# ViliamVadocz/takzero

Hardware: AMD Instinct MI355X
Metric: mcts_simulations_per_s (higher is better)
Workload: dtype f16

## Files before the change

### takzero_amd/csrc/tz_nn.hip

```cpp
#include "tz_nn.h"
#include "tz_fp8.h"
#include "tz_fp6.h"
#include <type_traits>
#include "tz_ot.h"

#include <algorithm>
#include <cmath>
#include <cstdio>
#include <cstdlib>
#include <cstring>
#include <atomic>
#include <map>
#include <memory>
#include <mutex>
#include <thread>

int tz_nn_launch_split(int sp, int n, const void* net_args, int max_positions, hipStream_t st);
int tz_nn_launch_c6(int n, const void* net_args, int max_positions, hipStream_t st);
size_t tz_nn_c6_seed_bytes(int n, int max_positions);

namespace {

typedef float f32x4 __attribute__((ext_vector_type(4)));
typedef unsigned int u32x4 __attribute__((ext_vector_type(4)));
// ... 2623 lines not shown
                                const float wv = W(co, ci, t);
                                const _Float16 hi = (_Float16)wv;
                                const size_t at = (((((size_t)t * m_total + mh) * ct_total + ct) * 2) * 64 + lane) * 32 + i;
                                p8[at] = tz_f32_to_e4m3((wv - (float)hi) * 2048.0f * sw);
                                p8[at + 64 * 32] = tz_f32_to_e4m3((float)hi * sw);
                            }
                        }
            if ((rc = upload(p8, &L->w8))) return rc;
        }
        if (with_c6) {
            if (L->cin_pad % 128) return tz_fail(TZ_EINVAL, "weights: TZ_PREC_F16C6 needs input channels in multiples of 128");
            const int g_total = L->cin_pad / 128;
            constexpr size_t REC = 3328;
            std::vector<unsigned char> p6((size_t)taps * g_total * ct_total * REC, 0);
            for (int t = 0; t < taps; t++)
                for (int g = 0; g < g_total; g++)
                    for (int ct = 0; ct < ct_total; ct++) {
                        unsigned char* rec = p6.data() + (((size_t)t * g_total + g) * ct_total + ct) * REC;
                        for (int lane = 0; lane < 64; lane++) {
                            const int co = ct * 16 + (lane & 15), q = lane >> 4;
                            float lo[32], hi[32], amax_l = 0.0f, amax_h = 0.0f;
                            for (int i = 0; i < 32; i++) {
                                const int ci = 128 * g + 32 * (i >> 3) + 8 * q + (i & 7);
                                const float wv = (co < cout && ci < cin) ? W(co, ci, t) : 0.0f;
                                const _Float16 h = (_Float16)wv;
                                hi[i] = (float)h;
                                lo[i] = wv - (float)h;
                                amax_h = std::max(amax_h, fabsf(hi[i]));
                                amax_l = std::max(amax_l, fabsf(lo[i]));
                            }
                            const uint32_t bl = tz_e2m3_block_scale_byte(amax_l), bh = tz_e2m3_block_scale_byte(amax_h);
                            uint8_t cl[32], ch[32];
                            for (int i = 0; i < 32; i++) {
                                cl[i] = tz_f32_to_e2m3(ldexpf(lo[i], 127 - (int)bl));
                                ch[i] = tz_f32_to_e2m3(ldexpf(hi[i], 127 - (int)bh));
                            }
                            uint32_t sl[6], sh[6];
                            tz_pack_fp6x32(cl, sl);
                            tz_pack_fp6x32(ch, sh);
                            memcpy(rec + 0 * 1536 + lane * 16, sl, 16);
                            memcpy(rec + 0 * 1536 + 1024 + lane * 8, sl + 4, 8);
                            memcpy(rec + 1 * 1536 + lane * 16, sh, 16);
                            memcpy(rec + 1 * 1536 + 1024 + lane * 8, sh + 4, 8);
                            const uint32_t sw = bl | (bh << 8);
                            memcpy(rec + 3072 + lane * 4, &sw, 4);
                        }
                    }
            if ((rc = upload(p6, &L->w8))) return rc;
        }
        return upload(p, &L->w_mfma);
    }
    std::vector<float> f((size_t)taps * cin * cout);
    for (int t = 0; t < taps; t++)
        for (int ci = 0; ci < cin; ci++)
            for (int co = 0; co < cout; co++) f[((size_t)t * cin + ci) * cout + co] = W(co, ci, t);
    return upload(f, &L->w_f32);
}

void free_layer(ConvW* L) {
    if (L->w_mfma) (void)hipFree(L->w_mfma);
    if (L->w_lo) (void)hipFree(L->w_lo);
    if (L->w8) (void)hipFree(L->w8);
    if (L->w_f32) (void)hipFree(L->w_f32);
    if (L->bias) (void)hipFree(L->bias);
    *L = ConvW();
}

int bn_fold(const TensorMap& m, const std::string& p, int c, std::vector<float>& scale, std::vector<float>& bias) {
    std::vector<float> g, b, mean, var;
    int rc;
    if ((rc = get_tensor(m, p + ".weight", c, g))) return rc;
    if ((rc = get_tensor(m, p + ".bias", c, b))) return rc;
    if ((rc = get_tensor(m, p + ".running_mean", c, mean))) return rc;
    if ((rc = get_tensor(m, p + ".running_var", c, var))) return rc;
    scale.resize(c);
    bias.resize(c);
    for (int i = 0; i < c; i++) {
        const float s = g[i] / sqrtf(var[i] + 1e-5f);
        scale[i] = s;
        bias[i] = b[i] - mean[i] * s;
    }
    return TZ_OK;
}

struct NetWeights {
    ConvW conv_in, policy;
    std::vector<ConvW> res;
    uint16_t* tower_w = nullptr;
    uint16_t* tower_w_lo = nullptr;
    unsigned char* tower_w8 = nullptr;
    float* c8_scales = nullptr;
    float* tower_bias = nullptr;
    float* heads = nullptr;
    ConvW rnd[2][3];
    uint16_t* rndw[3] = {nullptr, nullptr, nullptr};
    float* rndb[3] = {nullptr, nullptr, nullptr};
    float rnd_min = 0.f, rnd_max = 1.f;
    float* simhash = nullptr;
};

void free_weights(NetWeights& w) {
    free_layer(&w.conv_in);
    free_layer(&w.policy);
    for (auto& l : w.res) free_layer(&l);
    w.res.clear();
    if (w.tower_w) (void)hipFree(w.tower_w);
    if (w.tower_w_lo) (void)hipFree(w.tower_w_lo);
    if (w.tower_w8) (void)hipFree(w.tower_w8);
    if (w.c8_scales) (void)hipFree(w.c8_scales);
    if (w.tower_bias) (void)hipFree(w.tower_bias);
    w.tower_w = nullptr;
    w.tower_w_lo = nullptr;
    w.tower_w8 = nullptr;
    w.c8_scales = nullptr;
    w.tower_bias = nullptr;
    if (w.heads) (void)hipFree(w.heads);
    w.heads = nullptr;
    for (int a = 0; a < 2; a++)
        for (int b = 0; b < 3; b++) free_layer(&w.rnd[a][b]);
    for (int l = 0; l < 3; l++) {
        if (w.rndw[l]) (void)hipFree(w.rndw[l]);
        if (w.rndb[l]) (void)hipFree(w.rndb[l]);
        w.rndw[l] = nullptr;
        w.rndb[l] = nullptr;
    }
    if (w.simhash) (void)hipFree(w.simhash);
    w.simhash = nullptr;
}

int build_weights(tz_net* net, const TensorMap& m, NetWeights& W) {
    const int nn = net->nn, cin = net->cin, prec = net->precision;
    std::vector<float> w, scale, bias;
    int rc;
    if ((rc = get_tensor(m, "core.input_conv2d.weight", (size_t)FILTERS * cin * 9, w))) return rc;
    if ((rc = bn_fold(m, "core.batch_norm", FILTERS, scale, bias))) return rc;
    const bool split = prec == TZ_PREC_F16X2, c8 = prec == TZ_PREC_F16C8, c6 = prec == TZ_PREC_F16C6;
    std::vector<int> c6_perm(FILTERS);
    for (int pos = 0; pos < FILTERS; pos++) c6_perm[pos] = c6_channel_at(pos);
    const std::vector<int>* tower_perm = c6 ? &c6_perm : nullptr;
    if ((rc = build_layer(prec, 9, cin, FILTERS, 256, w, scale, bias, nullptr, &W.conv_in, split || c8 || c6))) return rc;
    W.res.resize(2 * net->blocks);
    {
        const int nl = 2 * net->blocks;
        const int workers = std::max(1, std::min(nl, std::min(16, (int)std::thread::hardware_concurrency())));
        std::atomic<int> next{0}, failed{TZ_OK};
        std::string first_error;
        std::mutex mu;
        const bool background = g_upload_stream != nullptr;
        auto work = [&]() {
            if (hipSetDevice(net->device) != hipSuccess) {
                failed = TZ_EDEVICE;
                return;
            }
            std::unique_ptr<UploadStream> upload_stream(background ? new UploadStream() : nullptr);
            if (upload_stream && !upload_stream->mine) {
                std::lock_guard<std::mutex> lk(mu);
                if (failed == TZ_OK) {
                    failed = TZ_EDEVICE;
                    first_error = "weights: cannot create an upload stream for a build thread";
                }
                return;
            }
            std::vector<float> lw, lscale, lbias;
            for (int l = next++; l < nl && failed == TZ_OK; l = next++) {
                const std::string p = "core.res_block_" + std::to_string(l / 2) + ((l & 1) ? ".b" : ".a");
                int r = get_tensor(m, p + ".conv2d.weight", (size_t)FILTERS * FILTERS * 9, lw);
                if (!r) r = bn_fold(m, p + ".batch_norm", FILTERS, lscale, lbias);
                if (!r) r = build_layer(prec, 9, FILTERS, FILTERS, 256, lw, lscale, lbias, tower_perm, &W.res[l], split, c8, c6);
                if (r) {
                    std::lock_guard<std::mutex> lk(mu);
                    if (failed == TZ_OK) {
                        failed = r;
                        first_error = tz_last_error();
                    }
                }
            }
        };
        std::vector<std::thread> pool;
        for (int t = 1; t < workers; t++) pool.emplace_back(work);
        work();
        for (auto& t : pool) t.join();
        if (failed != TZ_OK) return tz_fail(failed, first_error.empty() ? "weights: a tower layer could not be built" : first_error);
    }
    if (prec != TZ_PREC_F32 && net->blocks > 0) {
        const size_t layer_elems = (size_t)9 * 8 * 16 * 64 * 8, nl = W.res.size();
        TZ_HIP(hipMalloc(&W.tower_w, nl * layer_elems * 2));
        if (split) TZ_HIP(hipMalloc(&W.tower_w_lo, nl * layer_elems * 2));
        const size_t layer_bytes8 = c6 ? (size_t)9 * 2 * 16 * 3328 : (size_t)9 * 2 * 16 * 2 * 64 * 32;
        if (c8 || c6) TZ_HIP(hipMalloc(&W.tower_w8, nl * layer_bytes8));
        TZ_HIP(hipMalloc(&W.tower_bias, nl * FILTERS * sizeof(float)));
        for (size_t l = 0; l < nl; l++) {
            if ((rc = copy_sync(W.tower_w + l * layer_elems, W.res[l].w_mfma, layer_elems * 2, hipMemcpyDeviceToDevice))) return rc;
            if (split && (rc = copy_sync(W.tower_w_lo + l * layer_elems, W.res[l].w_lo, layer_elems * 2, hipMemcpyDeviceToDevice))) return rc;
            if ((c8 || c6) && (rc = copy_sync(W.tower_w8 + l * layer_bytes8, W.res[l].w8, layer_bytes8, hipMemcpyDeviceToDevice))) return rc;
            if ((rc = copy_sync(W.tower_bias + l * FILTERS, W.res[l].bias, FILTERS * sizeof(float), hipMemcpyDeviceToDevice))) return rc;
        }
    }
    if ((rc = get_tensor(m, "policy.conv2d.weight", (size_t)net->pol_ch * FILTERS * 9, w))) return rc;
    if ((rc = get_tensor(m, "policy.conv2d.bias", net->pol_ch, bias))) return rc;
    if ((rc = build_layer(prec, 9, FILTERS, net->pol_ch, net->pol_stride, w, {}, bias, tower_perm, &W.policy, split, c8, c6))) return rc;
    if (c8) {
        std::vector<float> cs;
        for (auto& l : W.res) cs.push_back(l.c8_scale);
        cs.push_back(W.policy.c8_scale);
        if ((rc = upload(cs, &W.c8_scales))) return rc;
    }
    std::vector<float> hv, hu, lv, lu, t1;
    if ((rc = get_tensor(m, "value.conv2d.weight", FILTERS, hv))) return rc;
    if ((rc = get_tensor(m, "ube.conv2d.weight", FILTERS, hu))) return rc;
    if ((rc = get_tensor(m, "value.linear.weight", nn, lv))) return rc;
    if ((rc = get_tensor(m, "ube.linear.weight", nn, lu))) return rc;
    std::vector<float> hw;
    hw.insert(hw.end(), hv.begin(), hv.end());
    hw.insert(hw.end(), hu.begin(), hu.end());
    hw.insert(hw.end(), lv.begin(), lv.end());
    hw.insert(hw.end(), lu.begin(), lu.end());
    for (const char* nm : {"value.conv2d.bias", "ube.conv2d.bias", "value.linear.bias", "ube.linear.bias"}) {
        if ((rc = get_tensor(m, nm, 1, t1))) return rc;
        hw.push_back(t1[0]);
    }
    if ((rc = upload(hw, &W.heads))) return rc;
    if (net->has_rnd) {
        const int in_size = cin * nn;
        std::vector<int> perm(in_size);
        for (int px = 0; px < nn; px++)
            for (int c = 0; c < cin; c++) perm[px * cin + c] = c * nn + px;
        const char* nets[2] = {"rnd_learning", "rnd_target"};
        const char* layers[3] = {"input_linear", "hidden_linear", "final_linear"};
        const int dims[4] = {in_size, 1024, 1024, 512};
        for (int a = 0; a < 2; a++)
            for (int l = 0; l < 3; l++) {
                const std::string p = std::string(nets[a]) + "." + layers[l];
                if ((rc = get_tensor(m, p + ".weight", (size_t)dims[l + 1] * dims[l], w))) return rc;
                if ((rc = get_tensor(m, p + ".bias", dims[l + 1], bias))) return rc;
                if ((rc = build_layer(prec, 1, dims[l], dims[l + 1], 256, w, {}, bias, l == 0 ? &perm : nullptr, &W.rnd[a][l])))
                    return rc;
            }
        if (prec != TZ_PREC_F32) {
            std::vector<float> wa, wb, ba, bb;
            if ((rc = get_tensor(m, "rnd_learning.input_linear.weight", (size_t)1024 * in_size, wa))) return rc;
            if ((rc = get_tensor(m, "rnd_target.input_linear.weight", (size_t)1024 * in_size, wb))) return rc;
            if ((rc = get_tensor(m, "rnd_learning.input_linear.bias", 1024, ba))) return rc;
            if ((rc = get_tensor(m, "rnd_target.input_linear.bias", 1024, bb))) return rc;
            wa.insert(wa.end(), wb.begin(), wb.end());
            ba.insert(ba.end(), bb.begin(), bb.end());
            ConvW cat;
            if ((rc = build_layer(prec, 1, in_size, 2048, 256, wa, {}, ba, &perm, &cat))) return rc;
            W.rndw[0] = cat.w_mfma;
            W.rndb[0] = cat.bias;
            for (int l = 1; l < 3; l++) {
                const size_t welems = (size_t)(W.rnd[0][l].cin_pad / 32) * (W.rnd[0][l].cout_pad / 16) * 512;
                const size_t belems = W.rnd[0][l].cout_pad;
                TZ_HIP(hipMalloc(&W.rndw[l], 2 * welems * 2));
                TZ_HIP(hipMalloc(&W.rndb[l], 2 * belems * sizeof(float)));
                for (int a = 0; a < 2; a++) {
                    if ((rc = copy_sync(W.rndw[l] + a * welems, W.rnd[a][l].w_mfma, welems * 2, hipMemcpyDeviceToDevice))) return rc;
                    if ((rc = copy_sync(W.rndb[l] + a * belems, W.rnd[a][l].bias, belems * sizeof(float), hipMemcpyDeviceToDevice))) return rc;
                }
            }
        }
        if ((rc = get_tensor(m, "min", 1, t1))) return rc;
        W.rnd_min = t1[0];
        if ((rc = get_tensor(m, "max", 1, t1))) return rc;
        W.rnd_max = t1[0];
    }
    if (net->has_hash) {
        if ((rc = get_tensor(m, "simhash_matrix", (size_t)cin * nn * 32, w))) return rc;
        if ((rc = upload(w, &W.simhash))) return rc;
    }
    return TZ_OK;
}

__host__ __device__ constexpr int ppt_small(int nb) { return nb == 1 ? 64 : nb == 3 ? 7 : nb == 4 ? 6 : nb == 5 ? 4 : 3; }

int conv_cfg() {
    static int cfg = -1;
    if (cfg < 0) {
        const char* e = getenv("TZ_CONV_CFG");
        cfg = e ? atoi(e) : 0;
    }
    return cfg;
}

template <int NB, int P, int NW, int RN, int TAPS, bool FROM_STATE, bool SINGLE, int ABL = 0, int LAYOUT = 1, typename ET = __bf16, int OCC = 2>
int launch_conv(const ConvArgs& a, int max_positions, int n_blocks_y, hipStream_t st) {
    constexpr int NN = NB * NB, RT = (P * NN + 15) / 16, LROWS = RT * 16 + 8;
    const size_t smem = LdsImg<LAYOUT>::bytes(LROWS);
    auto kern = conv_mfma_kernel<NB, P, RN, TAPS, FROM_STATE, ABL, SINGLE, NW, LAYOUT, ET, OCC>;
    static bool attr_done[64] = {};
    int attr_dev = 0;
    TZ_HIP(hipGetDevice(&attr_dev));
    bool& attr_set = attr_done[attr_dev & 63];
    if (!attr_set) {
        TZ_HIP(hipFuncSetAttribute(reinterpret_cast<const void*>(kern), hipFuncAttributeMaxDynamicSharedMemorySize, (int)smem));
        attr_set = true;
    }
    dim3 grid((max_positions + P - 1) / P, n_blocks_y, a.groups > 1 ? a.groups : 1);
    hipLaunchKernelGGL(kern, grid, dim3(NW * 64), smem, st, a);
    hipError_t e = hipGetLastError();
    if (e != hipSuccess) return tz_fail(TZ_EDEVICE, std::string("conv launch: ") + hipGetErrorString(e));
    return TZ_OK;
}

int linear_grouped_bf16(int precision, const uint16_t* w, const float* bias, int groups, int cin_pad, int cout_pad, const void* in,
                        int in_stride, int in_z, void* out, int out_stride, int out_z, bool relu, bool out_f32,
                        const int32_t* count_dev, int count_host, int max_positions, hipStream_t st) {
    ConvArgs a;
    memset(&a, 0, sizeof a);
    a.in = in;
    a.count_dev = count_dev;
    a.count_host = count_host;
    a.w = w;
    a.bias = bias;
    a.out = out;
    a.cin_pad = cin_pad;
    a.kc_total = cin_pad / 32;
    a.ct_total = cout_pad / 16;
    a.out_stride = out_stride;
    a.cin_real = cin_pad;
    a.relu = relu;
    a.out_f32 = out_f32;
    a.in_stride = in_stride;
    a.groups = groups;
    a.in_z = in_z;
    a.w_z_frags = a.kc_total * a.ct_total;
    a.bias_z = cout_pad;
    a.out_z = out_z;
    if (max_positions <= 128) {
        if (prec_is_f16(precision)) return launch_conv<1, 32, 8, 2, 1, false, false, 0, 1, _Float16>(a, max_positions, cout_pad / 256, st);
        return launch_conv<1, 32, 8, 2, 1, false, false>(a, max_positions, cout_pad / 256, st);
    }
    if (prec_is_f16(precision)) return launch_conv<1, 128, 8, 2, 1, false, false, 0, 1, _Float16>(a, max_positions, cout_pad / 256, st);
    return launch_conv<1, 128, 8, 2, 1, false, false>(a, max_positions, cout_pad / 256, st);
}

template <int NB, typename ET>
int conv_board(const ConvArgs& a, int cout_pad, bool from_state, int max_positions, hipStream_t st) {
    constexpr int PA = ppt_for(NB), PB = ppt_small(NB);
    const bool wide = cout_pad % 256 == 0;
    const int by = wide ? cout_pad / 256 : cout_pad / 128;
    if (conv_cfg() == 0) {
        if (from_state) return launch_conv<NB, PA, 8, 2, 9, true, false, 0, 1, ET>(a, max_positions, by, st);
        if (wide) return launch_conv<NB, PA, 8, 2, 9, false, true, 0, 1, ET>(a, max_positions, by, st);
        return launch_conv<NB, PA, 8, 1, 9, false, true, 0, 1, ET>(a, max_positions, by, st);
    }
    if (from_state) return launch_conv<NB, PB, 4, 4, 9, true, false, 0, 1, ET>(a, max_positions, by, st);
    if (wide) return launch_conv<NB, PB, 4, 4, 9, false, true, 0, 1, ET>(a, max_positions, by, st);
    return launch_conv<NB, PB, 4, 2, 9, false, true, 0, 1, ET>(a, max_positions, by, st);
}

template <typename ET>
int conv_dispatch(int n, bool board, const ConvArgs& a, int cout_pad, bool from_state, int max_positions, hipStream_t st) {
    if (!board) return launch_conv<1, 64, 8, 2, 1, false, false, 0, 1, ET>(a, max_positions, cout_pad / 256, st);
    switch (n) {
        case 3: return conv_board<3, ET>(a, cout_pad, from_state, max_positions, st);
        case 4: return conv_board<4, ET>(a, cout_pad, from_state, max_positions, st);
        case 5: return conv_board<5, ET>(a, cout_pad, from_state, max_positions, st);
        case 6: return conv_board<6, ET>(a, cout_pad, from_state, max_positions, st);
    }
    return tz_fail(TZ_EINVAL, "conv: unsupported board size");
}

int conv_bf16(tz_net* net, const ConvW& L, const void* in, const tz_state* states, const int32_t* gidx,
              const int32_t* count_dev, int count_host, int max_positions, const void* residual, void* out,
              int out_stride, bool relu, bool out_f32, bool board, hipStream_t st) {
    ConvArgs a;
    a.in = in;
    a.states = states;
    a.game_index = gidx;
    a.count_dev = count_dev;
    a.count_host = count_host;
    a.w = L.w_mfma;
    a.bias = L.bias;
    a.residual = residual;
    a.out = out;
    a.cin_pad = L.cin_pad;
    a.kc_total = L.cin_pad / 32;
    a.ct_total = L.cout_pad / 16;
    a.out_stride = out_stride;
    a.cin_real = L.cin;
    a.relu = relu;
    a.out_f32 = out_f32;
    a.has_res = residual != nullptr;
    a.in_stride = L.cin_pad;
    a.groups = 1;
    a.in_z = a.w_z_frags = a.bias_z = a.out_z = 0;
    if (prec_is_f16(net->precision)) return conv_dispatch<_Float16>(net->n, board, a, L.cout_pad, in == nullptr, max_positions, st);
    return conv_dispatch<__bf16>(net->n, board, a, L.cout_pad, in == nullptr, max_positions, st);
}

#ifdef TZ_ABLATIONS
template <int NB>
int launch_tower4x2(const TowerArgs& a, int max_positions, hipStream_t st) {
    constexpr int P = ppt_for(NB), NN = NB * NB, RT = (P * NN + 15) / 16, LROWS = RT * 16 + 8;
    const size_t smem = (size_t)LROWS * LDS_ROWB * 8 + (size_t)9 * RT * 64 * 4;
    auto kern = tower4x2_mfma_kernel<NB, P>;
    static bool attr_done[64] = {};
    int attr_dev = 0;
    TZ_HIP(hipGetDevice(&attr_dev));
    bool& attr_set = attr_done[attr_dev & 63];
    if (!attr_set) {
        TZ_HIP(hipFuncSetAttribute(reinterpret_cast<const void*>(kern), hipFuncAttributeMaxDynamicSharedMemorySize, (int)smem));
        attr_set = true;
    }
    hipLaunchKernelGGL(kern, dim3((max_positions + P - 1) / P), dim3(512), smem, st, a);
    hipError_t e = hipGetLastError();
    if (e != hipSuccess) return tz_fail(TZ_EDEVICE, std::string("tower4x2 launch: ") + hipGetErrorString(e));
    return TZ_OK;
}
#endif

template <int NB, int OPT = 0, typename ET = __bf16>
int launch_tower(const TowerArgs& a, int max_positions, hipStream_t st) {
    constexpr int P = ppt_for(NB), NN = NB * NB, RT = (P * NN + 15) / 16, LROWS = RT * 16 + 8;
    const size_t smem = (size_t)LROWS * LDS_ROWB * 8 + ((OPT & 4096) ? (size_t)9 * RT * 64 * 4 : 0);
    auto kern = tower_mfma_kernel<NB, P, OPT, ET>;
    static bool attr_done[64] = {};
    int attr_dev = 0;
    TZ_HIP(hipGetDevice(&attr_dev));
    bool& attr_set = attr_done[attr_dev & 63];
    if (!attr_set) {
        TZ_HIP(hipFuncSetAttribute(reinterpret_cast<const void*>(kern), hipFuncAttributeMaxDynamicSharedMemorySize, (int)smem));
        attr_set = true;
    }
    hipLaunchKernelGGL(kern, dim3((max_positions + P - 1) / P), dim3(512), smem, st, a);
    hipError_t e = hipGetLastError();
    if (e != hipSuccess) return tz_fail(TZ_EDEVICE, std::string("tower launch: ") + hipGetErrorString(e));
    return TZ_OK;
}

int tower_bf16(tz_net* net, const void* in, void* out, const int32_t* count_dev, int count_host, int max_positions,
               hipStream_t st) {
    TowerArgs a;
    a.in = reinterpret_cast<const uint16_t*>(in);
    a.out = reinterpret_cast<uint16_t*>(out);
    a.w = net->tower_w;
    a.bias = net->tower_bias;
    a.count_dev = count_dev;
    a.count_host = count_host;
    a.nlayers = 2 * net->blocks;
    const bool h = prec_is_f16(net->precision);
    switch (net->n) {
        case 3: return h ? launch_tower<3, 4224, _Float16>(a, max_positions, st) : launch_tower<3, 4224>(a, max_positions, st);
        case 4: return h ? launch_tower<4, 4224, _Float16>(a, max_positions, st) : launch_tower<4, 4224>(a, max_positions, st);
        case 5: return h ? launch_tower<5, 4224, _Float16>(a, max_positions, st) : launch_tower<5, 4224>(a, max_positions, st);
        case 6: return h ? launch_tower<6, 4224, _Float16>(a, max_positions, st) : launch_tower<6, 4224>(a, max_positions, st);
    }
    return tz_fail(TZ_EINVAL, "tower: unsupported board size");
}

#endif

int net_fused_mode() {
    static int mode = -1;
    if (mode < 0) {
        const char* e = getenv("TZ_TOWER");
        mode = e ? atoi(e) : 2;
    }
    return mode;
}

constexpr int NET_SPLIT_MAX_GROUPS = 64;
constexpr size_t NET_SPLIT_PLANE_BYTES = 7680;
constexpr int NET_SPLIT_MAX_POSITIONS = 4 * NET_SPLIT_MAX_GROUPS;

template <int NB, int RNP, typename ET, bool PERM, int P = ppt_for(NB), int SP = 0, int ABL = 0, int TT = 0, int NW = 8, int SPLIT = 1>
int launch_net(const NetArgs& a, int max_positions, hipStream_t st) {
    constexpr int RT = RowMap<NB, P, PERM>::RT, LROWS = RT * 16 + 8;
    constexpr bool ROWTAB = SP != 0 && NB == 6 && P == 4;
    constexpr size_t tap_bytes = TT ? (size_t)9 * RT * RowMap<NB, P, PERM>::PPT * sizeof(int) : (size_t)9 * RT * 64 * (ROWTAB ? 1 : SP == 2 ? sizeof(uint16_t) : sizeof(int));
    constexpr size_t smem = (size_t)LROWS * LDS_ROWB * (SP == 2 ? (NB == 6 ? 16 : 20) : SP ? 16 : 8) + 2 * RT * 16 * sizeof(float) + tap_bytes + (SPLIT > 1 ? 16 : 0);
    static_assert(smem <= 160 * 1024, "net kernel: the LDS image does not fit a CU");
    auto kern = net_mfma_kernel<NB, P, RNP, ET, PERM, SP, ABL, TT, NW, SPLIT>;
    static bool attr_done[64] = {};
    int attr_dev = 0;
    TZ_HIP(hipGetDevice(&attr_dev));
    bool& attr_set = attr_done[attr_dev & 63];
    if (!attr_set) {
        TZ_HIP(hipFuncSetAttribute(reinterpret_cast<const void*>(kern), hipFuncAttributeMaxDynamicSharedMemorySize, (int)smem));
        attr_set = true;
    }
    int blocks = (max_positions + P - 1) / P;
    if (SPLIT > 1) {
        const int groups = (blocks + 7) / 8 * 8;
        if (groups > NET_SPLIT_MAX_GROUPS || !a.xch || !a.xch_count) return tz_fail(TZ_EINVAL, "net launch: the several-CU form is for small batches");
        TZ_HIP(hipMemsetAsync(a.xch_count, 0, (size_t)groups * 128, st));
        blocks = groups * SPLIT;
    }
    hipLaunchKernelGGL(kern, dim3(blocks), dim3(NW * 64), smem, st, a);
    hipError_t e = hipGetLastError();
    if (e != hipSuccess) return tz_fail(TZ_EDEVICE, std::string("net launch: ") + hipGetErrorString(e));
    return TZ_OK;
}

bool net_square_major() {
    static int v = -1;
    if (v < 0) {
        const char* e = getenv("TZ_NET_ROWS");
        v = (e && !strcmp(e, "board")) ? 0 : 1;
    }
    return v == 1;
}

int net_small_p(int max_positions) {
    static const bool full = getenv("TZ_NET_P") && !strcmp(getenv("TZ_NET_P"), "full");
    if (full) return 0;
    return max_positions <= 256 ? 1 : max_positions <= 512 ? 2 : max_positions <= 1024 ? 4 : 0;
}

#if defined(TZ_NN_C6_TU)
}
#elif defined(TZ_NN_SPLIT_TU)
}

int tz_nn_launch_split(int sp, int n, const void* net_args, int max_positions, hipStream_t st) {
    const NetArgs& a = *static_cast<const NetArgs*>(net_args);
    if (sp == 1) {
        if (n == 5 && a.xch && max_positions <= NET_SPLIT_MAX_POSITIONS) {
            if (max_positions <= NET_SPLIT_MAX_GROUPS) return launch_net<5, 1, _Float16, false, 1, 1, 0, 0, 4, 4>(a, max_positions, st);
            if (max_positions <= 2 * NET_SPLIT_MAX_GROUPS) return launch_net<5, 1, _Float16, false, 2, 1, 0, 0, 4, 4>(a, max_positions, st);
            return launch_net<5, 1, _Float16, false, 4, 1, 0, 0, 4, 4>(a, max_positions, st);
        }
        switch (n) {
            case 3: return launch_net<3, 1, _Float16, false, 8, 1>(a, max_positions, st);
            case 4: return launch_net<4, 1, _Float16, false, 6, 1>(a, max_positions, st);
            case 5: return launch_net<5, 1, _Float16, true, 4, 1>(a, max_positions, st);
            case 6:
                if (net_square_major() && max_positions >= 1024) return launch_net<6, 2, _Float16, true, 4, 1>(a, max_positions, st);
                return launch_net<6, 2, _Float16, false, 2, 1>(a, max_positions, st);
        }
        return tz_fail(TZ_EINVAL, "net: unsupported board size");
    }
#ifdef TZ_ABLATIONS
    if (n == 5 && getenv("TZ_NET_ABL") && atoi(getenv("TZ_NET_ABL")) == 16) return launch_net<5, 1, _Float16, true, 4, 2, 16>(a, max_positions, st);
    if (n == 5 && getenv("TZ_NET_ABL") && atoi(getenv("TZ_NET_ABL")) == 32) return launch_net<5, 1, _Float16, true, 4, 2, 32>(a, max_positions, st);
    if (n == 5 && getenv("TZ_NET_ABL") && atoi(getenv("TZ_NET_ABL")) == 48) return launch_net<5, 1, _Float16, true, 4, 2, 48>(a, max_positions, st);
#endif
    if (n == 5 && net_small_p(max_positions) == 1) return launch_net<5, 1, _Float16, false, 1, 2>(a, max_positions, st);
    if (n == 5 && net_small_p(max_positions) == 2) return launch_net<5, 1, _Float16, false, 2, 2>(a, max_positions, st);
    switch (n) {
        case 3: return launch_net<3, 1, _Float16, false, 8, 2>(a, max_positions, st);
        case 4: return launch_net<4, 1, _Float16, false, 6, 2>(a, max_positions, st);
        case 5: return launch_net<5, 1, _Float16, true, 4, 2>(a, max_positions, st);
        case 6:
            if (net_square_major() && max_positions >= 1024) return launch_net<6, 2, _Float16, true, 4, 2>(a, max_positions, st);
            return launch_net<6, 2, _Float16, false, 2, 2>(a, max_positions, st);
    }
    return tz_fail(TZ_EINVAL, "net: unsupported board size");
}
#else

bool net_p6_four() {
    static const bool four = getenv("TZ_NET_P6") && !strcmp(getenv("TZ_NET_P6"), "4");
    return four;
}

template <typename ET>
int net_fused_et(tz_net* net, const NetArgs& a, int max_positions, hipStream_t st) {
    const bool sq = net_square_major();
    const int small = net_small_p(max_positions);
    if (net->n == 5 && a.xch && max_positions <= NET_SPLIT_MAX_POSITIONS && sizeof(ET) == 2) {
        if (max_positions <= NET_SPLIT_MAX_GROUPS) return launch_net<5, 1, ET, false, 1, 0, 0, 0, 4, 4>(a, max_positions, st);
        if (max_positions <= 2 * NET_SPLIT_MAX_GROUPS) return launch_net<5, 1, ET, false, 2, 0, 0, 0, 4, 4>(a, max_positions, st);
        return launch_net<5, 1, ET, false, 4, 0, 0, 0, 4, 4>(a, max_positions, st);
    }
    if (net->n == 4 && a.xch && max_positions <= 2 * NET_SPLIT_MAX_GROUPS && sizeof(ET) == 2) {
        if (max_positions <= NET_SPLIT_MAX_GROUPS) return launch_net<4, 1, ET, false, 1, 0, 0, 0, 4, 4>(a, max_positions, st);
        return launch_net<4, 1, ET, false, 2, 0, 0, 0, 4, 4>(a, max_positions, st);
    }
    if (net->n == 6 && a.xch && max_positions <= 2 * NET_SPLIT_MAX_GROUPS && sizeof(ET) == 2) {
        if (max_positions <= NET_SPLIT_MAX_GROUPS) return launch_net<6, 2, ET, false, 1, 0, 0, 0, 4, 4>(a, max_positions, st);
        return launch_net<6, 2, ET, false, 2, 0, 0, 0, 4, 4>(a, max_positions, st);
    }
    if (net->n == 5 && small == 1) return launch_net<5, 1, ET, false, 1>(a, max_positions, st);
    if (net->n == 5 && small == 2) return launch_net<5, 1, ET, false, 2>(a, max_positions, st);
    if (net->n == 5 && small == 4) return launch_net<5, 1, ET, false, 4>(a, max_positions, st);
    if (net->n == 6 && small == 1) return launch_net<6, 2, ET, false, 1>(a, max_positions, st);
    if (net->n == 6 && small == 2) return launch_net<6, 2, ET, false, 2>(a, max_positions, st);
#ifdef TZ_ABLATIONS
    if (const char* e = getenv("TZ_NET_ABL")) {
        if (net->n == 5 && sq && small == 0 && sizeof(ET) == 2) {
            switch (atoi(e)) {
                case 1: return launch_net<5, 1, ET, true, 8, 0, 1>(a, max_positions, st);
                case 2: return launch_net<5, 1, ET, true, 8, 0, 2>(a, max_positions, st);
                case 3: return launch_net<5, 1, ET, true, 8, 0, 3>(a, max_positions, st);
                case 4: return launch_net<5, 1, ET, true, 8, 0, 4>(a, max_positions, st);
                case 8: return launch_net<5, 1, ET, true, 8, 0, 8>(a, max_positions, st);
                case 16: return launch_net<5, 1, ET, true, 8, 0, 16>(a, max_positions, st);
                case 32: return launch_net<5, 1, ET, true, 8, 0, 32>(a, max_positions, st);
                case 48: return launch_net<5, 1, ET, true, 8, 0, 48>(a, max_positions, st);
                case 64: return launch_net<5, 1, ET, true, 8, 0, 64>(a, max_positions, st);
                case 80: return launch_net<5, 1, ET, true, 8, 0, 80>(a, max_positions, st);
                default: break;
            }
        }
    }
#endif
    switch (net->n) {
        case 3: return sq ? launch_net<3, 1, ET, true>(a, max_positions, st) : launch_net<3, 1, ET, false>(a, max_positions, st);
        case 4: return launch_net<4, 1, ET, false>(a, max_positions, st);
        case 5:
#ifdef TZ_ABLATIONS
            if (sq && getenv("TZ_NET_TT") && atoi(getenv("TZ_NET_TT")) == 1) return launch_net<5, 1, ET, true, 8, 0, 0, 1>(a, max_positions, st);
#endif
#ifdef TZ_ABLATIONS
            if (sq && getenv("TZ_NET_W4") && atoi(getenv("TZ_NET_W4")) == 1) return launch_net<5, 1, ET, true, 8, 0, 0, 0, 4>(a, max_positions, st);
#endif
            return sq ? launch_net<5, 1, ET, true>(a, max_positions, st) : launch_net<5, 1, ET, false>(a, max_positions, st);
        case 6:
            if (sq && max_positions >= 2048 && !net_p6_four()) return launch_net<6, 2, ET, true, 8, 0, 0, 1>(a, max_positions, st);
            return sq ? launch_net<6, 2, ET, true>(a, max_positions, st) : launch_net<6, 2, ET, false>(a, max_positions, st);
    }
    return tz_fail(TZ_EINVAL, "net: unsupported board size");
}

bool net_fused_writes_rnd_input(const tz_net* net) {
    static const bool separate = getenv("TZ_RND_PREP_KERNEL") != nullptr;
    if (net->eval_split) return false;
    return !separate && net->has_rnd && net->n == 5 && net->cin % 8 == 0 && (net->cin * net->nn) % 32 == 0;
}

int net_fused(tz_net* net, const tz_state* states, const int32_t* gidx, const int32_t* count_dev, int count_host,
              int max_positions, hipStream_t st) {
    NetArgs a;
    a.states = states;
    a.game_index = gidx;
    a.count_dev = count_dev;
    a.count_host = count_host;
    a.w_in = net->conv_in.w_mfma;
    a.bias_in = net->conv_in.bias;
    a.cin_real = net->conv_in.cin;
    a.kc_in = net->conv_in.cin_pad / 32;
    a.w = net->tower_w;
    a.bias = net->tower_bias;
    a.nlayers = 2 * net->blocks;
    a.w_pol = net->policy.w_mfma;
// ... 1193 lines not shown
```

Measured before the change: 1.450 million.

## Add dedicated pipelined MFMA linear kernel with occupancy-aware row tiling

Adds a specialised linear (1x1) MFMA kernel that double-buffers 256-channel input slices in LDS, keeps a ring of prefetched weight fragments in registers, and uses LDS-only barriers. It replaces the generic conv kernel for large-batch grouped linears. When too few workgroups would cover the CUs it uses 64-row tiles instead of 128 to raise parallelism. An env var can restore the old conv path. The gain relies on overlapping global loads with MFMA; the cost is more register pressure and a new, complex code path.

```diff
diff --git a/takzero_amd/csrc/tz_nn.hip b/takzero_amd/csrc/tz_nn.hip
--- a/takzero_amd/csrc/tz_nn.hip
+++ b/takzero_amd/csrc/tz_nn.hip
@@ -2949,6 +2949,147 @@
     return TZ_OK;
 }
 
+__device__ __forceinline__ void lds_only_barrier() { asm volatile("s_waitcnt lgkmcnt(0)\n\ts_barrier" ::: "memory"); }
+
+template <int P, typename ET>
+__global__ __launch_bounds__(512, 2) void linear_mfma_kernel(ConvArgs a) {
+    typedef typename Elem<ET>::x8 ex8;
+    typedef typename Elem<ET>::x4 ex4;
+    constexpr int NW = 8, NT = NW * 64, RN = 2, RT = P / 16, RING = 4;
+    constexpr int PLANE = P * LDS_ROWB, BUF = PLANE * 8;
+    constexpr int NLOAD = P * 32 / NT;
+    static_assert(P % 16 == 0 && (P * 32) % NT == 0 && (RT - 1) * 16 * LDS_ROWB + 7 * PLANE < 65536, "tile");
+    extern __shared__ __attribute__((aligned(16))) unsigned char lds[];
+    const int count = a.count_dev ? *a.count_dev : a.count_host;
+    const int pos0 = blockIdx.x * P;
+    if (pos0 >= count) return;
+    const int tid = threadIdx.x, lane = tid & 63;
+    const int wave = __builtin_amdgcn_readfirstlane(tid >> 6);
+    const int q = lane >> 4, lr = lane & 15;
+    const int valid_rows = min(P, count - pos0);
+    const size_t m0 = (size_t)pos0;
+    const int ct0 = (blockIdx.y * NW + wave) * RN;
+    const __amdgpu_buffer_rsrc_t wrsrc = __builtin_amdgcn_make_buffer_rsrc(
+        const_cast<uint16_t*>(a.w), 0, (a.groups > 1 ? a.groups * a.w_z_frags : a.kc_total * a.ct_total) * 1024, 0x00020000);
+    const int lane16 = lane * 16;
+    const int frag0 = (int)blockIdx.z * a.w_z_frags + ct0;
+    auto wload = [&](int kt, int j) __attribute__((always_inline)) -> ex8 {
+        const u32x4 r = __builtin_amdgcn_raw_buffer_load_b128(wrsrc, lane16, (frag0 + kt * a.ct_total + j) * 1024, 0);
+        return __builtin_bit_cast(ex8, r);
+    };
+    const int KT = a.kc_total, nslices = (KT + 7) / 8;
+    const uint16_t* in = reinterpret_cast<const uint16_t*>(a.in) + (size_t)blockIdx.z * a.in_z;
+    u32x4 stage[NLOAD];
+    auto fetch_slice = [&](int slice) __attribute__((always_inline)) {
+        const int cpr = min(256, a.cin_pad - slice * 256) / 8;
+#pragma unroll
+        for (int i = 0; i < NLOAD; i++) {
+            const int id = tid + i * NT, row = min(id >> 5, valid_rows - 1), ci = min(id & 31, cpr - 1);
+            stage[i] = *reinterpret_cast<const u32x4*>(in + (m0 + row) * a.in_stride + slice * 256 + ci * 8);
+        }
+    };
+    auto store_slice = [&](int buf) __attribute__((always_inline)) {
+#pragma unroll
+        for (int i = 0; i < NLOAD; i++) {
+            const int id = tid + i * NT, row = id >> 5, ci = id & 31;
+            *reinterpret_cast<u32x4*>(lds + buf + LdsImg<1>::store_addr(row, ci, PLANE)) = stage[i];
+        }
+    };
+    fetch_slice(0);
+    ex8 bq[RING][RN];
+#pragma unroll
+    for (int d = 0; d < RING - 1; d++)
+#pragma unroll
+        for (int j = 0; j < RN; j++) bq[d][j] = wload(min(d, KT - 1), j);
+    store_slice(0);
+    fetch_slice(min(1, nslices - 1));
+    lds_only_barrier();
+    __builtin_amdgcn_sched_barrier(0);
+    f32x4 acc[RT][RN];
+#pragma unroll
+    for (int rt = 0; rt < RT; rt++)
+#pragma unroll
+        for (int j = 0; j < RN; j++) acc[rt][j] = f32x4{0.f, 0.f, 0.f, 0.f};
+    const int abase = lr * LDS_ROWB + lds_piece(lr, q);
+    ex8 av[RT];
+#pragma unroll
+    for (int rt = 0; rt < RT; rt++) av[rt] = *reinterpret_cast<const ex8*>(lds + abase + rt * 16 * LDS_ROWB);
+    auto slice_body = [&](int s, auto fetch_c, auto next_c) __attribute__((always_inline)) {
+        constexpr bool FETCH = decltype(fetch_c)::value, NEXT = decltype(next_c)::value;
+        const int kcs = NEXT ? 8 : KT - s * 8;
+        const int cb = abase + (s & 1) * BUF, ob = abase + BUF - (s & 1) * BUF;
+#pragma unroll
+        for (int kc = 0; kc < 8; kc++) {
+            if (!NEXT && kc >= kcs) break;
+#pragma unroll
+            for (int j = 0; j < RN; j++) bq[(kc + RING - 1) % RING][j] = wload(min(s * 8 + kc + RING - 1, KT - 1), j);
+            if (NEXT && kc == 1) {
+                store_slice(BUF - (s & 1) * BUF);
+                if (FETCH) fetch_slice(s + 2);
+            }
+            if (NEXT && kc == 7) lds_only_barrier();
+            __builtin_amdgcn_sched_barrier(0);
+            const bool wrap = NEXT ? kc == 7 : kc + 1 >= kcs;
+            const int rb = wrap ? (NEXT ? ob : cb) : cb + (kc + 1) * PLANE;
+#pragma unroll
+            for (int rt = 0; rt < RT; rt++) {
+#pragma unroll
+                for (int j = 0; j < RN; j++) acc[rt][j] = Elem<ET>::mfma(bq[kc % RING][j], av[rt], acc[rt][j]);
+                av[rt] = *reinterpret_cast<const ex8*>(lds + rb + rt * 16 * LDS_ROWB);
+            }
+        }
+    };
+    int s = 0;
+    if (nslices > 2) slice_body(s++, std::true_type{}, std::true_type{});
+    for (; s + 2 < nslices; s++) slice_body(s, std::true_type{}, std::true_type{});
+    if (s + 1 < nslices) slice_body(s++, std::false_type{}, std::true_type{});
+    slice_body(s, std::false_type{}, std::false_type{});
+
+#pragma unroll
+    for (int j = 0; j < RN; j++) {
+        const int cbase = (ct0 + j) * 16 + q * 4;
+        const f32x4 bias = *reinterpret_cast<const f32x4*>(a.bias + (size_t)blockIdx.z * a.bias_z + cbase);
+#pragma unroll
+        for (int rt = 0; rt < RT; rt++) {
+            const int r = rt * 16 + lr;
+            if (r >= valid_rows) continue;
+            f32x4 v = acc[rt][j] + bias;
+            const size_t o = (size_t)blockIdx.z * a.out_z + (m0 + r) * a.out_stride + cbase;
+            if (a.relu) {
+#pragma unroll
+                for (int k = 0; k < 4; k++) v[k] = v[k] > 0.f ? v[k] : 0.f;
+            }
+            if (a.out_f32) {
+                *reinterpret_cast<f32x4*>(reinterpret_cast<float*>(a.out) + o) = v;
+            } else {
+                ex4 ov;
+#pragma unroll
+                for (int k = 0; k < 4; k++) ov[k] = Elem<ET>::cvt(v[k]);
+                *reinterpret_cast<ex4*>(reinterpret_cast<uint16_t*>(a.out) + o) = ov;
+            }
+        }
+    }
+}
+
+template <int P, typename ET>
+int launch_linear(const ConvArgs& a, int max_positions, int n_blocks_y, hipStream_t st) {
+    const size_t smem = 2 * (size_t)P * LDS_ROWB * 8;
+    auto kern = linear_mfma_kernel<P, ET>;
+    static bool attr_done[64] = {};
+    int attr_dev = 0;
+    TZ_HIP(hipGetDevice(&attr_dev));
+    bool& attr_set = attr_done[attr_dev & 63];
+    if (!attr_set) {
+        TZ_HIP(hipFuncSetAttribute(reinterpret_cast<const void*>(kern), hipFuncAttributeMaxDynamicSharedMemorySize, (int)smem));
+        attr_set = true;
+    }
+    dim3 grid((max_positions + P - 1) / P, n_blocks_y, a.groups > 1 ? a.groups : 1);
+    hipLaunchKernelGGL(kern, grid, dim3(512), smem, st, a);
+    hipError_t e = hipGetLastError();
+    if (e != hipSuccess) return tz_fail(TZ_EDEVICE, std::string("linear launch: ") + hipGetErrorString(e));
+    return TZ_OK;
+}
+
 int linear_grouped_bf16(int precision, const uint16_t* w, const float* bias, int groups, int cin_pad, int cout_pad, const void* in,
                         int in_stride, int in_z, void* out, int out_stride, int out_z, bool relu, bool out_f32,
                         const int32_t* count_dev, int count_host, int max_positions, hipStream_t st) {
@@ -2977,8 +3118,26 @@
         if (prec_is_f16(precision)) return launch_conv<1, 32, 8, 2, 1, false, false, 0, 1, _Float16>(a, max_positions, cout_pad / 256, st);
         return launch_conv<1, 32, 8, 2, 1, false, false>(a, max_positions, cout_pad / 256, st);
     }
-    if (prec_is_f16(precision)) return launch_conv<1, 128, 8, 2, 1, false, false, 0, 1, _Float16>(a, max_positions, cout_pad / 256, st);
-    return launch_conv<1, 128, 8, 2, 1, false, false>(a, max_positions, cout_pad / 256, st);
+    static const int mode = [] {
+        const char* e = getenv("TZ_RND_LINEAR");
+        return !e ? 0 : !strcmp(e, "conv") ? 1 : !strcmp(e, "rows128") ? 2 : 0;
+    }();
+    if (mode == 1) {
+        if (prec_is_f16(precision)) return launch_conv<1, 128, 8, 2, 1, false, false, 0, 1, _Float16>(a, max_positions, cout_pad / 256, st);
+        return launch_conv<1, 128, 8, 2, 1, false, false>(a, max_positions, cout_pad / 256, st);
+    }
+    static int cus[64] = {};
+    int dev = 0;
+    TZ_HIP(hipGetDevice(&dev));
+    int& ncu = cus[dev & 63];
+    if (!ncu) TZ_HIP(hipDeviceGetAttribute(&ncu, hipDeviceAttributeMultiprocessorCount, dev));
+    const int wg128 = (max_positions + 127) / 128 * (cout_pad / 256) * (groups > 1 ? groups : 1);
+    if (mode != 2 && wg128 < ncu) {
+        if (prec_is_f16(precision)) return launch_linear<64, _Float16>(a, max_positions, cout_pad / 256, st);
+        return launch_linear<64, __bf16>(a, max_positions, cout_pad / 256, st);
+    }
+    if (prec_is_f16(precision)) return launch_linear<128, _Float16>(a, max_positions, cout_pad / 256, st);
+    return launch_linear<128, __bf16>(a, max_positions, cout_pad / 256, st);
 }
 
 template <int NB, typename ET>
```

Result: no change. 1.449 million (-0.0%).
